# Baozhi888/distributed-gpu-inference

Hardware: AMD Instinct MI355X
Metric: output tokens/sec (node) + p50 TTFT, Llama-3-70B P/D-split layer-pipeline 8 GPU [this run: 1-GPU run, layout single, model llama3-70b (not the P/D-split headline layout)] (higher is better)
Workload: dtype bf16

## Files before the change

### dgi/csrc/decode_attention.hip

```cpp
#include <type_traits>

#include "common.h"

using namespace dgi;

namespace {

constexpr int kRsrcWord3 = 0x00020000;
constexpr int kSc1 = 16;

template <int HD>
__device__ __forceinline__ int v_lds_off(int row, int col) {
  constexpr int NCH = HD / 8;
  const int ch = (col >> 3) ^ (((row & 7) << 1) & (NCH - 1));
  return row * HD + (ch << 3) + (col & 7);
}

__device__ __forceinline__ int o_swz(int q) { return ((q & 3) << 3) | (q >> 2); }

template <int HD>
constexpr int decode_wave_lds() {
  return (32 * HD * 2 > 16 * (HD + 4) * 4 ? 32 * HD * 2 : 16 * (HD + 4) * 4) + 128;
}

struct DecodePlan {
  int base, nsplit, part;
};
template <bool WIN>
__device__ __forceinline__ DecodePlan decode_plan(int ctx, int window, int part_size, int max_splits) {
  DecodePlan p;
  p.base = WIN ? (max(0, ctx - window) & ~31) : 0;
  const int span = ctx - p.base;
  if (part_size > 0) {
    p.part = part_size;
    p.nsplit = (span + p.part - 1) / p.part;
  } else {
    p.nsplit = max(1, min(max_splits, (span + (-part_size) - 1) / (-part_size)));
    p.part = (((span + p.nsplit - 1) / p.nsplit) + 31) & ~31;
    p.nsplit = (span + p.part - 1) / p.part;
  }
  return p;
}

template <int HD, int NW, bool FP8, bool WIN, typename... S>
__global__ __launch_bounds__(64 * NW) void paged_decode_kernel(
    const uint16_t* __restrict__ q, int q_stride, const uint16_t* __restrict__ k_cache,
    const uint16_t* __restrict__ v_cache, const int* __restrict__ block_tables, int bt_stride,
    const int* __restrict__ context_lens, uint16_t* __restrict__ out, int out_stride,
    float* __restrict__ part_o, float* __restrict__ part_lse, int* __restrict__ counters, int max_splits, int nh,
    int nkv, int bs_log2, int part_size, float scale_log2, bool page16, S... extra) {
  constexpr int KS = HD / 32;
  constexpr int NC = HD / 16;
  constexpr int VCH = HD / 8;
  constexpr int WREG = decode_wave_lds<HD>();
  constexpr int OROW = HD;
  constexpr int NT = 64 * NW;
  extern __shared__ __attribute__((aligned(16))) char smem[];

  const int split = blockIdx.x;
  const int h = blockIdx.y;
  const int b = blockIdx.z;
  const int ctx = context_lens[b];
  [[maybe_unused]] float v_scale = 1.f;
  if constexpr (FP8) {
    const float* sc = pack_ptr(extra...);
    scale_log2 *= sc[h];
    v_scale = sc[nkv + h];
  }
  [[maybe_unused]] const uint8_t* k8 = reinterpret_cast<const uint8_t*>(k_cache);
  [[maybe_unused]] const uint8_t* v8 = reinterpret_cast<const uint8_t*>(v_cache);
  const __amdgpu_buffer_rsrc_t po_rs = __builtin_amdgcn_make_buffer_rsrc(
      (void*)part_o, 0, (int)min((size_t)gridDim.z * nh * max_splits * HD * 4, (size_t)0x7fffffff), kRsrcWord3);
  const __amdgpu_buffer_rsrc_t pl_rs = __builtin_amdgcn_make_buffer_rsrc(
      (void*)part_lse, 0, (int)min((size_t)gridDim.z * nh * max_splits * 4, (size_t)0x7fffffff), kRsrcWord3);
  int window = 0;
  if constexpr (WIN) window = pack_window(extra...);
  [[maybe_unused]] const int lo = max(0, ctx - window);
  const DecodePlan plan = decode_plan<WIN>(ctx, window, part_size, max_splits);
  const int nsplit = plan.nsplit, part = plan.part;
  const int start = plan.base + split * part;
  if (start >= ctx) return;
  const int end = min(start + part, ctx);
  const int G = nh / nkv;
  const int bs = 1 << bs_log2;

  const int tid = threadIdx.x;
  const int w = __builtin_amdgcn_readfirstlane(tid >> 6);
  const int lane = tid & 63;
  const int qi = lane & 15;
  const int g = lane >> 4;
  uint16_t* vt = reinterpret_cast<uint16_t*>(smem + w * WREG);

  u32x4 qf[KS];
  auto load_q = [&]() {
#pragma unroll
    for (int s = 0; s < KS; ++s) {
      if (qi < G) {
        qf[s] = *reinterpret_cast<const u32x4*>(q + (size_t)b * q_stride + (h * G + qi) * HD + 32 * s + 8 * g);
      } else {
        qf[s] = u32x4{0, 0, 0, 0};
      }
    }
  };
  constexpr bool LATE_Q = NW == 8;
  if (!LATE_Q) load_q();

  const int* bt = block_tables + (size_t)b * bt_stride;
  const size_t head_stride = (size_t)bs * HD;

  float m_run = -1e30f, l_run = 0.f;
  f32x4 o[NC];
#pragma unroll
  for (int c = 0; c < NC; ++c) o[c] = f32x4{0, 0, 0, 0};

  const int ntiles = (end - start + 31) >> 5;
  for (int t = w; t < ntiles; t += NW) {
    const int tb = start + (t << 5);
    using raw_t = typename std::conditional<FP8, uint2, u32x4>::type;
    raw_t kf[2][KS];
    raw_t vr[VCH / 2];
    if (page16 && tb + 32 <= end) {
      const int fb = tb >> 4;
      const uint16_t* kp[2];
      const uint16_t* vp[2];
#pragma unroll
      for (int j = 0; j < 2; ++j) {
        const size_t page = ((size_t)bt[fb + j] * nkv + h) * head_stride;
        kp[j] = k_cache + page;
        vp[j] = v_cache + page;
      }
#pragma unroll
      for (int u = 0; u < 2; ++u)
#pragma unroll
        for (int s = 0; s < KS; ++s) {
          if constexpr (FP8)
            kf[u][s] = *reinterpret_cast<const uint2*>(k8 + (kp[u] - k_cache) + qi * HD + 32 * s + 8 * g);
          else
            kf[u][s] = *reinterpret_cast<const u32x4*>(kp[u] + qi * HD + 32 * s + 8 * g);
        }
#pragma unroll
      for (int k = 0; k < VCH / 2; ++k) {
        const int idx = k * 64 + lane;
        const int row = idx / VCH;
        if constexpr (FP8)
          vr[k] = *reinterpret_cast<const uint2*>(v8 + (vp[row >> 4] - v_cache) + (row & 15) * HD + (idx % VCH) * 8);
        else
          vr[k] = *reinterpret_cast<const u32x4*>(vp[row >> 4] + (row & 15) * HD + (idx % VCH) * 8);
      }
    } else {
#pragma unroll
      for (int u = 0; u < 2; ++u) {
        int tok = tb + 16 * u + qi;
        tok = min(tok, end - 1);
        const int blk = bt[tok >> bs_log2];
        const uint16_t* kpl = k_cache + ((size_t)blk * nkv + h) * head_stride + (size_t)(tok & (bs - 1)) * HD;
#pragma unroll
        for (int s = 0; s < KS; ++s) {
          if constexpr (FP8) kf[u][s] = *reinterpret_cast<const uint2*>(k8 + (kpl - k_cache) + 32 * s + 8 * g);
          else kf[u][s] = *reinterpret_cast<const u32x4*>(kpl + 32 * s + 8 * g);
        }
      }
#pragma unroll
      for (int k = 0; k < VCH / 2; ++k) {
        const int idx = k * 64 + lane;
        const int row = idx / VCH;
        const int ch = idx % VCH;
        int tok = min(tb + row, end - 1);
        const int blk = bt[tok >> bs_log2];
        const uint16_t* vpl = v_cache + ((size_t)blk * nkv + h) * head_stride + (size_t)(tok & (bs - 1)) * HD;
        if constexpr (FP8) vr[k] = *reinterpret_cast<const uint2*>(v8 + (vpl - v_cache) + ch * 8);
        else vr[k] = *reinterpret_cast<const u32x4*>(vpl + ch * 8);
      }
    }
    if (LATE_Q && t == w) load_q();
    f32x4 sacc[2];
#pragma unroll
    for (int u = 0; u < 2; ++u) {
      sacc[u] = f32x4{0, 0, 0, 0};
#pragma unroll
      for (int s = 0; s < KS; ++s) {
        if constexpr (FP8)
          sacc[u] = __builtin_amdgcn_mfma_f32_16x16x32_bf16(widen8(kf[u][s].x, kf[u][s].y), as_bf16x8(qf[s]),
                                                            sacc[u], 0, 0, 0);
        else
          sacc[u] = __builtin_amdgcn_mfma_f32_16x16x32_bf16(as_bf16x8(kf[u][s]), as_bf16x8(qf[s]), sacc[u], 0, 0, 0);
      }
    }
    asm volatile("s_waitcnt lgkmcnt(0)" ::: "memory");
#pragma unroll
    for (int k = 0; k < VCH / 2; ++k) {
      const int idx = k * 64 + lane;
      const int row = idx / VCH;
      const int ch = idx % VCH;
      if constexpr (FP8) *reinterpret_cast<u32x4*>(vt + v_lds_off<HD>(row, ch * 8)) = widen8_u32(vr[k].x, vr[k].y);
      else *reinterpret_cast<u32x4*>(vt + v_lds_off<HD>(row, ch * 8)) = vr[k];
    }
    const bool full = tb + 32 <= end && !(WIN && tb < lo);
    float x[2][4];
    float mx = -1e30f;
    if (full) {
#pragma unroll
      for (int u = 0; u < 2; ++u)
#pragma unroll
        for (int i = 0; i < 4; ++i) {
          x[u][i] = sacc[u][i] * scale_log2;
          mx = fmaxf(mx, x[u][i]);
        }
    } else {
#pragma unroll
      for (int u = 0; u < 2; ++u)
#pragma unroll
        for (int i = 0; i < 4; ++i) {
          const int tok = tb + 16 * u + 4 * g + i;
          const bool vis = WIN ? (tok < end) & (tok >= lo) : tok < end;
          const float v = vis ? sacc[u][i] * scale_log2 : -1e30f;
          x[u][i] = v;
          mx = fmaxf(mx, v);
        }
    }
    mx = fmaxf(mx, __shfl_xor(mx, 16, 64));
    mx = fmaxf(mx, __shfl_xor(mx, 32, 64));
    const float m_new = fmaxf(m_run, mx);
    const float alpha = __builtin_amdgcn_exp2f(m_run - m_new);
    float psum = 0.f;
    float p[2][4];
#pragma unroll
    for (int u = 0; u < 2; ++u)
#pragma unroll
      for (int i = 0; i < 4; ++i) {
        p[u][i] = __builtin_amdgcn_exp2f(x[u][i] - m_new);
        psum += p[u][i];
      }
    psum += __shfl_xor(psum, 16, 64);
    psum += __shfl_xor(psum, 32, 64);
    l_run = l_run * alpha + psum;
    m_run = m_new;
#pragma unroll
    for (int c = 0; c < NC; ++c) o[c] *= alpha;
    u32x4 pf;
    pf[0] = pack_bf16x2(p[0][0], p[0][1]);
    pf[1] = pack_bf16x2(p[0][2], p[0][3]);
    pf[2] = pack_bf16x2(p[1][0], p[1][1]);
    pf[3] = pack_bf16x2(p[1][2], p[1][3]);
    asm volatile("s_waitcnt lgkmcnt(0)" ::: "memory");
    __builtin_amdgcn_wave_barrier();
    const int tq = qi >> 2, tp = qi & 3;
#pragma unroll
    for (int c = 0; c < NC; ++c) {
      short4v lo = __builtin_amdgcn_ds_read_tr16_b64_v4i16(
          (lds_short4*)(vt + v_lds_off<HD>(4 * g + tq, 16 * c + 4 * tp)));
      short4v hi = __builtin_amdgcn_ds_read_tr16_b64_v4i16(
          (lds_short4*)(vt + v_lds_off<HD>(16 + 4 * g + tq, 16 * c + 4 * tp)));
      u32x4 vf;
      vf[0] = (uint32_t)(uint16_t)lo[0] | ((uint32_t)(uint16_t)lo[1] << 16);
      vf[1] = (uint32_t)(uint16_t)lo[2] | ((uint32_t)(uint16_t)lo[3] << 16);
      vf[2] = (uint32_t)(uint16_t)hi[0] | ((uint32_t)(uint16_t)hi[1] << 16);
      vf[3] = (uint32_t)(uint16_t)hi[2] | ((uint32_t)(uint16_t)hi[3] << 16);
      o[c] = __builtin_amdgcn_mfma_f32_16x16x32_bf16(as_bf16x8(vf), as_bf16x8(pf), o[c], 0, 0, 0);
    }
  }

  __syncthreads();
  constexpr int MLOFF = WREG - 128;
  float* ow = reinterpret_cast<float*>(smem + w * WREG);
  float* ml = reinterpret_cast<float*>(smem + w * WREG + MLOFF);
  if (qi < G) {
#pragma unroll
    for (int c = 0; c < NC; ++c)
#pragma unroll
      for (int i = 0; i < 4; ++i) ow[qi * OROW + ((16 * c + 4 * g + i) ^ o_swz(qi))] = o[c][i];
    if (g == 0) {
      ml[qi] = m_run;
      ml[16 + qi] = l_run;
    }
  }
  __syncthreads();
  for (int idx = tid; idx < G * HD; idx += NT) {
    const int qq = idx / HD;
    const int d = idx - qq * HD;
    float M = -1e30f;
#pragma unroll
    for (int ww = 0; ww < NW; ++ww) M = fmaxf(M, reinterpret_cast<float*>(smem + ww * WREG + MLOFF)[qq]);
    float L = 0.f, acc = 0.f;
#pragma unroll
    for (int ww = 0; ww < NW; ++ww) {
      const float* mlw = reinterpret_cast<float*>(smem + ww * WREG + MLOFF);
      const float sc = exp2f(mlw[qq] - M);
      L += mlw[16 + qq] * sc;
      acc += reinterpret_cast<float*>(smem + ww * WREG)[qq * OROW + (d ^ o_swz(qq))] * sc;
    }
    const int head = h * G + qq;
    float r = acc / L;
    if constexpr (FP8) r *= v_scale;
    if (nsplit == 1) {
      out[(size_t)b * out_stride + head * HD + d] = f32_to_bf16(r);
    } else if (counters != nullptr) {
      const size_t pi = ((size_t)b * nh + head) * max_splits + split;
      __builtin_amdgcn_raw_buffer_store_b32(__builtin_bit_cast(uint32_t, r), po_rs,
                                            (int)((pi * HD + d) * 4), 0, kSc1);
      if (d == 0)
        __builtin_amdgcn_raw_buffer_store_b32(__builtin_bit_cast(uint32_t, M + log2f(L)), pl_rs, (int)(pi * 4), 0,
                                              kSc1);
    } else {
      const size_t pi = ((size_t)b * nh + head) * max_splits + split;
      part_o[pi * HD + d] = r;
      if (d == 0) part_lse[pi] = M + log2f(L);
    }
  }
  if (nsplit == 1 || counters == nullptr) return;
  __shared__ int s_last;
  asm volatile("s_waitcnt vmcnt(0)" ::: "memory");
  __syncthreads();
  if (tid == 0) {
    const int ticket = __hip_atomic_fetch_add(&counters[b * nkv + h], 1, __ATOMIC_RELAXED, __HIP_MEMORY_SCOPE_AGENT);
    const int last = ticket == nsplit - 1;
    if (last) {
      __builtin_amdgcn_fence(__ATOMIC_ACQUIRE, "agent");
      asm volatile("s_waitcnt vmcnt(0)" ::: "memory");
      __hip_atomic_store(&counters[b * nkv + h], 0, __ATOMIC_RELAXED, __HIP_MEMORY_SCOPE_AGENT);
    }
    s_last = last;
  }
  __syncthreads();
  if (!s_last) return;
  for (int idx = tid; idx < G * HD; idx += NT) {
    const int qq = idx / HD;
    const int d = idx - qq * HD;
    const int head = h * G + qq;
    const size_t base = ((size_t)b * nh + head) * max_splits;
    float M = -1e30f;
    for (int sp = 0; sp < nsplit; ++sp) M = fmaxf(M, part_lse[base + sp]);
    float W = 0.f, acc = 0.f;
    for (int sp = 0; sp < nsplit; ++sp) {
      const float wgt = exp2f(part_lse[base + sp] - M);
      W += wgt;
      acc += wgt * part_o[(base + sp) * HD + d];
    }
    out[(size_t)b * out_stride + head * HD + d] = f32_to_bf16(acc / W);
  }
}

template <int HD, bool WIN, typename... S>
__global__ __launch_bounds__(HD) void decode_reduce_kernel(
    const float* __restrict__ part_o, const float* __restrict__ part_lse,
    const int* __restrict__ context_lens, uint16_t* __restrict__ out, int out_stride, int max_splits,
    int nh, int part_size, S... extra) {
  const int b = blockIdx.x;
  const int head = blockIdx.y;
  const int ctx = context_lens[b];
  int window = 0;
  if constexpr (WIN) window = pack_window(extra...);
  const int nsplit = decode_plan<WIN>(ctx, window, part_size, max_splits).nsplit;
  if (nsplit <= 1) return;
  const size_t base = ((size_t)b * nh + head) * max_splits;
  float M = -1e30f;
  for (int s = 0; s < nsplit; ++s) M = fmaxf(M, part_lse[base + s]);
  float W = 0.f, acc = 0.f;
  for (int s = 0; s < nsplit; ++s) {
    const float wgt = exp2f(part_lse[base + s] - M);
    W += wgt;
    acc += wgt * part_o[(base + s) * HD + threadIdx.x];
  }
  out[(size_t)b * out_stride + head * HD + threadIdx.x] = f32_to_bf16(acc / W);
}

}

extern "C" int dgi_paged_decode(const void* q, int q_stride, const void* k_cache,
                                const void* v_cache, const int* block_tables, int bt_stride,
                                const int* context_lens, void* out, int out_stride, float* part_o,
                                float* part_lse, int* counters, int B, int nh, int nkv, int hd, int block_size,
                                int max_splits, int part_size, float scale, const float* kv_scale,
                                int window, hipStream_t s) {
  if (window < 0) return -6;
  if (B == 0) return 0;
  if (nh % nkv || nh / nkv > 16) return -2;
  if ((part_size > 0 && part_size % 128) || (part_size <= 0 && (part_size == 0 || (-part_size) % 32))) return -3;
  if (max_splits <= 1) counters = nullptr;
  if ((size_t)B * nh * max_splits * hd * 4 >= ((size_t)1 << 31)) counters = nullptr;
  int bs_log2 = 0;
  while ((1 << bs_log2) < block_size) ++bs_log2;
  if ((1 << bs_log2) != block_size) return -4;
  const float scale_log2 = scale * 1.4426950408889634f;
  static const bool page16_on = [] {
    const char* e = getenv("DGI_DECODE_PAGE16");
    return !(e && e[0] == '0');
  }();
  const bool page16 = page16_on && bs_log2 == 4;
  dim3 grid(max_splits, nkv, B);
  const bool wide = max_splits == 1 && B * nkv <= 128;
#define DGI_DECODE_ARGS                                                                                  \
  (const uint16_t*)q, q_stride, (const uint16_t*)k_cache, (const uint16_t*)v_cache, block_tables,        \
      bt_stride, context_lens, (uint16_t*)out, out_stride, part_o, part_lse, counters, max_splits, nh,   \
      nkv, bs_log2, part_size, scale_log2, page16
#define DGI_DECODE_CFG(HDV, NWV) <<<grid, 64 * NWV, NWV * decode_wave_lds<HDV>(), s>>>
#define DGI_DECODE(HDV, NWV)                                                                             \
  do {                                                                                                   \
    if (window > 0 && kv_scale)                                                                          \
      paged_decode_kernel<HDV, NWV, true, true, int, const float*> DGI_DECODE_CFG(HDV, NWV)(             \
          DGI_DECODE_ARGS, window, kv_scale);                                                            \
    else if (window > 0)                                                                                 \
      paged_decode_kernel<HDV, NWV, false, true, int> DGI_DECODE_CFG(HDV, NWV)(DGI_DECODE_ARGS, window); \
    else if (kv_scale)                                                                                   \
      paged_decode_kernel<HDV, NWV, true, false, const float*> DGI_DECODE_CFG(HDV, NWV)(DGI_DECODE_ARGS, \
                                                                                        kv_scale);       \
    else                                                                                                 \
      paged_decode_kernel<HDV, NWV, false, false> DGI_DECODE_CFG(HDV, NWV)(DGI_DECODE_ARGS);             \
  } while (0)
#define DGI_DECODE_REDUCE(HDV)                                                                           \
  do {                                                                                                   \
    if (window > 0)                                                                                      \
      decode_reduce_kernel<HDV, true, int><<<dim3(B, nh), HDV, 0, s>>>(                                  \
          part_o, part_lse, context_lens, (uint16_t*)out, out_stride, max_splits, nh, part_size, window); \
    else                                                                                                 \
      decode_reduce_kernel<HDV, false><<<dim3(B, nh), HDV, 0, s>>>(                                      \
          part_o, part_lse, context_lens, (uint16_t*)out, out_stride, max_splits, nh, part_size);        \
  } while (0)
  if (hd == 128) {
    if (wide) DGI_DECODE(128, 8);
    else DGI_DECODE(128, 4);
    DGI_CHECK_LAUNCH();
    if (max_splits > 1 && counters == nullptr) {
      DGI_DECODE_REDUCE(128);
      DGI_CHECK_LAUNCH();
    }
  } else if (hd == 64) {
    if (wide) DGI_DECODE(64, 8);
    else DGI_DECODE(64, 4);
    DGI_CHECK_LAUNCH();
    if (max_splits > 1 && counters == nullptr) {
      DGI_DECODE_REDUCE(64);
      DGI_CHECK_LAUNCH();
    }
  } else {
    return -5;
  }
#undef DGI_DECODE
#undef DGI_DECODE_REDUCE
#undef DGI_DECODE_CFG
#undef DGI_DECODE_ARGS
  return 0;
}
```

Baseline: 1880.

## Software-pipeline K/V loads across tiles in paged decode attention

Restructures the paged decode loop so the next tile's K and V registers are loaded as soon as the current tile's K (after the QK MFMAs) and V (after the LDS store) are consumed. Block-table page lookups are prefetched one tile further ahead. The goal is to hide global-memory latency behind compute. It also reorders the V LDS store indexing and adds a waves_per_eu(3) hint. The hint caps register use, which risks spills, and the register reuse depends on the compiler scheduling the loads correctly.

```diff
diff --git a/dgi/csrc/decode_attention.hip b/dgi/csrc/decode_attention.hip
--- a/dgi/csrc/decode_attention.hip
+++ b/dgi/csrc/decode_attention.hip
@@ -43,7 +43,7 @@
 }
 
 template <int HD, int NW, bool FP8, bool WIN, typename... S>
-__global__ __launch_bounds__(64 * NW) void paged_decode_kernel(
+__global__ __launch_bounds__(64 * NW) __attribute__((amdgpu_waves_per_eu(3))) void paged_decode_kernel(
     const uint16_t* __restrict__ q, int q_stride, const uint16_t* __restrict__ k_cache,
     const uint16_t* __restrict__ v_cache, const int* __restrict__ block_tables, int bt_stride,
     const int* __restrict__ context_lens, uint16_t* __restrict__ out, int out_stride,
@@ -52,6 +52,8 @@
   constexpr int KS = HD / 32;
   constexpr int NC = HD / 16;
   constexpr int VCH = HD / 8;
+  constexpr int VPER = VCH / 8;
+  static_assert(VPER >= 1 && VPER * (64 / VCH) == 8, "V passes must tile 8-row groups");
   constexpr int WREG = decode_wave_lds<HD>();
   constexpr int OROW = HD;
   constexpr int NT = 64 * NW;
@@ -114,30 +116,51 @@
   for (int c = 0; c < NC; ++c) o[c] = f32x4{0, 0, 0, 0};
 
   const int ntiles = (end - start + 31) >> 5;
-  for (int t = w; t < ntiles; t += NW) {
-    const int tb = start + (t << 5);
-    using raw_t = typename std::conditional<FP8, uint2, u32x4>::type;
+  using raw_t = typename std::conditional<FP8, uint2, u32x4>::type;
+  struct TileRegs {
     raw_t kf[2][KS];
     raw_t vr[VCH / 2];
+  };
+  auto tile_pages = [&](int tb, int (&pg)[2]) {
+    const int fb = tb >> 4;
+    pg[0] = bt[fb];
+    pg[1] = bt[fb + 1];
+  };
+  auto load_k = [&](int tb, const int (&pg)[2], TileRegs& r) {
+    auto& kf = r.kf;
     if (page16 && tb + 32 <= end) {
-      const int fb = tb >> 4;
-      const uint16_t* kp[2];
-      const uint16_t* vp[2];
-#pragma unroll
-      for (int j = 0; j < 2; ++j) {
-        const size_t page = ((size_t)bt[fb + j] * nkv + h) * head_stride;
-        kp[j] = k_cache + page;
-        vp[j] = v_cache + page;
-      }
-#pragma unroll
-      for (int u = 0; u < 2; ++u)
+#pragma unroll
+      for (int u = 0; u < 2; ++u) {
+        const uint16_t* kp = k_cache + ((size_t)pg[u] * nkv + h) * head_stride;
 #pragma unroll
         for (int s = 0; s < KS; ++s) {
           if constexpr (FP8)
-            kf[u][s] = *reinterpret_cast<const uint2*>(k8 + (kp[u] - k_cache) + qi * HD + 32 * s + 8 * g);
+            kf[u][s] = *reinterpret_cast<const uint2*>(k8 + (kp - k_cache) + qi * HD + 32 * s + 8 * g);
           else
-            kf[u][s] = *reinterpret_cast<const u32x4*>(kp[u] + qi * HD + 32 * s + 8 * g);
+            kf[u][s] = *reinterpret_cast<const u32x4*>(kp + qi * HD + 32 * s + 8 * g);
         }
+      }
+    } else {
+#pragma unroll
+      for (int u = 0; u < 2; ++u) {
+        int tok = tb + 16 * u + qi;
+        tok = min(tok, end - 1);
+        const int blk = bt[tok >> bs_log2];
+        const uint16_t* kpl = k_cache + ((size_t)blk * nkv + h) * head_stride + (size_t)(tok & (bs - 1)) * HD;
+#pragma unroll
+        for (int s = 0; s < KS; ++s) {
+          if constexpr (FP8) kf[u][s] = *reinterpret_cast<const uint2*>(k8 + (kpl - k_cache) + 32 * s + 8 * g);
+          else kf[u][s] = *reinterpret_cast<const u32x4*>(kpl + 32 * s + 8 * g);
+        }
+      }
+    }
+  };
+  auto load_v = [&](int tb, const int (&pg)[2], TileRegs& r) {
+    auto& vr = r.vr;
+    if (page16 && tb + 32 <= end) {
+      const uint16_t* vp[2];
+#pragma unroll
+      for (int j = 0; j < 2; ++j) vp[j] = v_cache + ((size_t)pg[j] * nkv + h) * head_stride;
 #pragma unroll
       for (int k = 0; k < VCH / 2; ++k) {
         const int idx = k * 64 + lane;
@@ -148,18 +171,6 @@
           vr[k] = *reinterpret_cast<const u32x4*>(vp[row >> 4] + (row & 15) * HD + (idx % VCH) * 8);
       }
     } else {
-#pragma unroll
-      for (int u = 0; u < 2; ++u) {
-        int tok = tb + 16 * u + qi;
-        tok = min(tok, end - 1);
-        const int blk = bt[tok >> bs_log2];
-        const uint16_t* kpl = k_cache + ((size_t)blk * nkv + h) * head_stride + (size_t)(tok & (bs - 1)) * HD;
-#pragma unroll
-        for (int s = 0; s < KS; ++s) {
-          if constexpr (FP8) kf[u][s] = *reinterpret_cast<const uint2*>(k8 + (kpl - k_cache) + 32 * s + 8 * g);
-          else kf[u][s] = *reinterpret_cast<const u32x4*>(kpl + 32 * s + 8 * g);
-        }
-      }
 #pragma unroll
       for (int k = 0; k < VCH / 2; ++k) {
         const int idx = k * 64 + lane;
@@ -172,7 +183,10 @@
         else vr[k] = *reinterpret_cast<const u32x4*>(vpl + ch * 8);
       }
     }
-    if (LATE_Q && t == w) load_q();
+  };
+  auto tile_math = [&](int tb, const TileRegs& r, auto&& k_free, auto&& v_free) {
+    auto& kf = r.kf;
+    auto& vr = r.vr;
     f32x4 sacc[2];
 #pragma unroll
     for (int u = 0; u < 2; ++u) {
@@ -186,15 +200,15 @@
           sacc[u] = __builtin_amdgcn_mfma_f32_16x16x32_bf16(as_bf16x8(kf[u][s]), as_bf16x8(qf[s]), sacc[u], 0, 0, 0);
       }
     }
+    k_free();
     asm volatile("s_waitcnt lgkmcnt(0)" ::: "memory");
 #pragma unroll
     for (int k = 0; k < VCH / 2; ++k) {
-      const int idx = k * 64 + lane;
-      const int row = idx / VCH;
-      const int ch = idx % VCH;
-      if constexpr (FP8) *reinterpret_cast<u32x4*>(vt + v_lds_off<HD>(row, ch * 8)) = widen8_u32(vr[k].x, vr[k].y);
-      else *reinterpret_cast<u32x4*>(vt + v_lds_off<HD>(row, ch * 8)) = vr[k];
-    }
+      uint16_t* dst = vt + v_lds_off<HD>((k % VPER) * (64 / VCH) + lane / VCH, (lane % VCH) * 8) + (k / VPER) * 8 * HD;
+      if constexpr (FP8) *reinterpret_cast<u32x4*>(dst) = widen8_u32(vr[k].x, vr[k].y);
+      else *reinterpret_cast<u32x4*>(dst) = vr[k];
+    }
+    v_free();
     const bool full = tb + 32 <= end && !(WIN && tb < lo);
     float x[2][4];
     float mx = -1e30f;
@@ -258,6 +272,29 @@
       vf[3] = (uint32_t)(uint16_t)hi[2] | ((uint32_t)(uint16_t)hi[3] << 16);
       o[c] = __builtin_amdgcn_mfma_f32_16x16x32_bf16(as_bf16x8(vf), as_bf16x8(pf), o[c], 0, 0, 0);
     }
+  };
+  auto full16 = [&](int t) { return page16 && start + (t << 5) + 32 <= end; };
+  auto none = [] {};
+  TileRegs r;
+  int pg[2] = {0, 0};
+  int t = w;
+  if (t < ntiles) {
+    if (full16(t)) tile_pages(start + (t << 5), pg);
+    load_k(start + (t << 5), pg, r);
+    load_v(start + (t << 5), pg, r);
+    if (LATE_Q) load_q();
+    if (t + NW < ntiles && full16(t + NW)) tile_pages(start + ((t + NW) << 5), pg);
+    for (; t + NW < ntiles; t += NW) {
+      const int tn = t + NW;
+      const int tbn = start + (tn << 5);
+      tile_math(
+          start + (t << 5), r, [&] { load_k(tbn, pg, r); },
+          [&] {
+            load_v(tbn, pg, r);
+            if (tn + NW < ntiles && full16(tn + NW)) tile_pages(tbn + (NW << 5), pg);
+          });
+    }
+    tile_math(start + (t << 5), r, none, none);
   }
 
   __syncthreads();
```

Result: no change. 1879, median of 3 (-0.1%).
